# ViliamVadocz/takzero

Hardware: AMD Instinct MI355X
Metric: mcts_simulations_per_s (higher is better)
Workload: dtype f16

## Files before the change

### takzero_amd/csrc/tz_capi.hip

```cpp
#include <algorithm>
#include <array>
#include <cmath>
#include <cstdlib>
#include <cstring>
#include <vector>

#include "tz_math.h"
#include "tz_nn.h"

struct tz_search {
    SearchDev d;
    tz_net* net = nullptr;
    int device = 0;
    hipStream_t stream = nullptr;
    bool own_stream = false;
    float* noise_dev = nullptr;
    int noise_cap = 0;
    uint16_t* act_dev = nullptr;
    int32_t* i32_dev = nullptr;
    int8_t* i8_dev = nullptr;
    tz_root_info* info_dev = nullptr;
    void* child_dev = nullptr;
    size_t child_cap = 0;
    hipGraphExec_t graph[2] = {nullptr, nullptr};
// ... 66 lines not shown
int one_simulation(tz_search* s, bool from_start) {
    const int gi = from_start ? 1 : 0;
    s->sim_index++;
    const bool sample = s->profile && (s->sim_index % 8 == 0);
    if (!s->use_graph || sample || s->warm[gi] < 2) {
        s->warm[gi]++;
        return one_simulation_eager(s, from_start, sample);
    }
    if (s->graph[gi] && s->net && s->graph_gen[gi] != s->net->weights_gen) {
        (void)hipGraphExecDestroy(s->graph[gi]);
        s->graph[gi] = nullptr;
    }
    if (!s->graph[gi]) {
        hipGraph_t g = nullptr;
        TZ_HIP(hipStreamBeginCapture(s->stream, hipStreamCaptureModeThreadLocal));
        const int rc = one_simulation_eager(s, from_start, false);
        const hipError_t e = hipStreamEndCapture(s->stream, &g);
        if (rc) {
            if (g) (void)hipGraphDestroy(g);
            return rc;
        }
        if (e != hipSuccess) return tz_fail(TZ_EDEVICE, std::string("hipStreamEndCapture: ") + hipGetErrorString(e));
        const hipError_t ei = hipGraphInstantiate(&s->graph[gi], g, nullptr, nullptr, 0);
        (void)hipGraphDestroy(g);
        if (ei != hipSuccess) return tz_fail(TZ_EDEVICE, std::string("hipGraphInstantiate: ") + hipGetErrorString(ei));
        s->graph_gen[gi] = s->net ? s->net->weights_gen : 0;
    }
    TZ_HIP(hipGraphLaunch(s->graph[gi], s->stream));
    return TZ_OK;
}

int one_simulation_eager(tz_search* s, bool from_start, bool profile) {
    int rc;
    hipEvent_t e0 = nullptr, e1 = nullptr, e2 = nullptr, e3 = nullptr;
    const bool saved_net_profile = s->net ? s->net->profile : false;
    if (s->net) s->net->profile = profile;
    struct Restore {
        tz_search* s;
        bool v;
        ~Restore() {
            if (s->net) s->net->profile = v;
        }
    } restore{s, saved_net_profile};
    if (profile) {
        TZ_HIP(hipEventCreate(&e0));
        TZ_HIP(hipEventCreate(&e1));
        TZ_HIP(hipEventCreate(&e2));
        TZ_HIP(hipEventCreate(&e3));
        TZ_HIP(hipEventRecord(e0, s->stream));
    }
    if ((rc = tz_tree_descend(s->d, from_start, s->stream))) return rc;
    if ((rc = tz_tree_compact_leaves(s->d, s->stream))) return rc;
    if (profile) TZ_HIP(hipEventRecord(e1, s->stream));
    NetOut out{nullptr, 0, nullptr, nullptr};
    if (s->d.agent_kind == TZ_AGENT_NET) {
        if ((rc = tz_net_forward_device(s->net, s->d.leaf_env, s->d.nn_game, s->d.nn_count, 0, s->d.batch, s->stream, &out)))
            return rc;
    }
    if (profile) TZ_HIP(hipEventRecord(e2, s->stream));
    if ((rc = tz_tree_expand(s->d, out, s->stream))) return rc;
    if (profile) {
        TZ_HIP(hipEventRecord(e3, s->stream));
        s->tree_events.push_back({e0, e1});
        s->tree_events.push_back({e2, e3});
        s->steps++;
    }
    return TZ_OK;
}

int ensure_noise(tz_search* s, int amax) {
    if ((size_t)amax * s->d.batch <= (size_t)s->noise_cap) return TZ_OK;
    if (s->noise_dev) (void)hipFree(s->noise_dev);
    s->noise_dev = nullptr;
    TZ_HIP(hipMalloc(&s->noise_dev, (size_t)amax * s->d.batch * sizeof(float)));
    s->noise_cap = amax * s->d.batch;
    return TZ_OK;
}

void free_leaf_batch(tz_search* s) {
    LeafBatchDev& b = s->lb;
    void* ptrs[] = {b.env, b.act, b.nact, b.traj, b.traj_len, b.logit, b.prob, b.value, b.variance, b.bad, b.count, b.forwards,
                    b.offset, b.index};
    for (void* p : ptrs)
        if (p) (void)hipFree(p);
    b = LeafBatchDev{};
    s->lb_slots = 0;
}

int ensure_leaf_batch(tz_search* s, int leaves) {
    const size_t slots = (size_t)s->d.batch * leaves;
    if (slots > s->lb_slots) {
        TZ_HIP(hipStreamSynchronize(s->stream));
        free_leaf_batch(s);
        LeafBatchDev& b = s->lb;
        const size_t amax = (size_t)s->d.max_actions;
        int rc = 0;
        rc |= dev_alloc(&b.env, slots);
        rc |= dev_alloc(&b.act, slots * amax);
        rc |= dev_alloc(&b.nact, slots);
        rc |= dev_alloc(&b.traj, slots * TZ_MAX_DEPTH);
        rc |= dev_alloc(&b.traj_len, slots);
        rc |= dev_alloc(&b.logit, slots * amax);
        rc |= dev_alloc(&b.prob, slots * amax);
        rc |= dev_alloc(&b.value, slots);
        rc |= dev_alloc(&b.variance, slots);
        rc |= dev_alloc(&b.bad, slots);
        rc |= dev_alloc(&b.count, s->d.batch);
        rc |= dev_alloc(&b.forwards, s->d.batch);
        rc |= dev_alloc(&b.offset, s->d.batch);
// ... 708 lines not shown
```

### takzero_amd/csrc/tz_engine.h

```cpp
#pragma once
#include <hip/hip_runtime.h>
#include <stdint.h>

#include <string>
#include <vector>

#include "../../include/takzero_hip.h"

#define TZ_MAX_DEPTH 512

void tz_set_error(const std::string& msg);
int tz_fail(int code, const std::string& msg);
#define TZ_HIP(call)                                                                              \
    do {                                                                                          \
        hipError_t _e = (call);                                                                   \
        if (_e != hipSuccess)                                                                     \
            return tz_fail(TZ_EDEVICE, std::string(#call) + ": " + hipGetErrorString(_e));       \
    } while (0)

struct TreeArrays {
    uint8_t* eval_tag;
    uint32_t* eval_bits;
    uint32_t* visits;
    float* prob;
// ... 2 lines not shown
    uint32_t* child0;
    uint16_t* nchild;
    uint16_t* action;
};

struct SearchDev {
    int batch, n, half_komi, cap, max_actions, agent_kind;
    int strict_capacity;
    int select_rule;
    TreeArrays t;
    uint8_t* bank;
    uint32_t* alloc;
    tz_state* env;
    float* betas;
    uint32_t* traj;
    uint32_t* traj_len;
    int32_t* start_node;
    uint8_t* leaf_kind;
    uint16_t* leaf_nact;
    uint16_t* leaf_act;
    tz_state* leaf_env;
    int32_t* nn_game;
    int32_t* nn_count;
    uint32_t* bfs_src;
    unsigned long long* counters;
    int32_t* error_flag;
    int8_t* term_reason;
    uint8_t* term_winner;
};

struct LeafBatchDev {
    int leaves;
    tz_state* env;
    uint16_t* act;
    uint16_t* nact;
    uint32_t* traj;
    uint32_t* traj_len;
    float* logit;
    float* prob;
    float* value;
    float* variance;
    uint8_t* bad;
    int32_t* count;
    int32_t* forwards;
    int32_t* offset;
    int32_t* index;
};

struct NetOut {
    const float* policy;
    int policy_stride;
    const float* value;
    const float* variance;
};

int tz_tree_descend(const SearchDev& s, bool from_start_nodes, hipStream_t st);
int tz_tree_compact_leaves(const SearchDev& s, hipStream_t st);
int tz_tree_expand(const SearchDev& s, const NetOut& out, hipStream_t st);
int tz_tree_apply_noise(const SearchDev& s, const float* noise_dev, int amax, float ratio, hipStream_t st);
int tz_tree_root_info(const SearchDev& s, tz_root_info* out_dev, hipStream_t st);
int tz_tree_root_children(const SearchDev& s, int amax, uint16_t* move_idx, uint32_t* visits, uint8_t* eval_tag,
                          uint32_t* eval_bits, float* logit, float* prob, float* std_dev, hipStream_t st);
int tz_tree_node(const SearchDev& s, int game, const uint16_t* path_dev, int len, uint32_t* out_words, int* status, int amax,
                 uint16_t* move_idx, uint32_t* visits, uint8_t* eval_tag, uint32_t* eval_bits, float* logit, float* prob, float* std_dev,
                 hipStream_t st);
int tz_tree_select_best(const SearchDev& s, uint16_t* out_dev, hipStream_t st);
int tz_tree_step(const SearchDev& s, const uint16_t* actions_dev, hipStream_t st);
int tz_tree_restart(const SearchDev& s, const int32_t* choice_dev, int8_t* terminal_dev, bool force_all,
                    bool with_opening_moves, hipStream_t st);
int tz_tree_reset_games(const SearchDev& s, const int32_t* idx_dev, int count, hipStream_t st);
int tz_tree_set_start_children(const SearchDev& s, const int32_t* child_index_dev, hipStream_t st);
int tz_tree_gumbel_root_fixup(const SearchDev& s, hipStream_t st);
int tz_tree_principal_variation(const SearchDev& s, int game, uint16_t* moves_dev, int cap, int* len_dev, hipStream_t st);
int tz_tree_descend_batch(const SearchDev& s, const LeafBatchDev& b, hipStream_t st);
int tz_tree_compact_batch(const SearchDev& s, const LeafBatchDev& b, hipStream_t st);
int tz_tree_expand_batch(const SearchDev& s, const LeafBatchDev& b, const NetOut& out, hipStream_t st);
int tz_tree_play_moves(const SearchDev& s, const uint16_t* actions_dev, int8_t* ok_dev, hipStream_t st);
```

### takzero_amd/csrc/tz_nn.h

```cpp
#pragma once
#include <string>
#include <vector>

#include "tz_engine.h"
#include "tz_ot.h"

struct ConvW {
    int taps = 0, cin = 0, cin_pad = 0, cout = 0, cout_pad = 0;
    uint16_t* w_mfma = nullptr;
    uint16_t* w_lo = nullptr;
    unsigned char* w8 = nullptr;
    float c8_scale = 0.0f;
    float* w_f32 = nullptr;
    float* bias = nullptr;
};

struct tz_net {
    int n = 0, nn = 0, arch = 0, device = 0, precision = 0, blocks = 0;
    int cin = 0, cin_pad = 0, pol_ch = 0, pol_stride = 0, ppt = 0;
    bool loaded = false, has_rnd = false, has_hash = false;
    TensorStore store;
    uint64_t weights_gen = 0;
    ConvW conv_in, policy;
    std::vector<ConvW> res;
    uint16_t* tower_w = nullptr;
    uint16_t* tower_w_lo = nullptr;
    unsigned char* tower_w8 = nullptr;
    float* c8_scales = nullptr;
    float* tower_bias = nullptr;
    float* heads = nullptr;
    ConvW rnd[2][3];
    uint16_t* rndw[3] = {nullptr, nullptr, nullptr};
    float* rndb[3] = {nullptr, nullptr, nullptr};
    float rnd_min = 0.0f, rnd_max = 1.0f;
    float* simhash = nullptr;
    uint32_t* bitset = nullptr;
    int max_batch = 0;
    void *act_a = nullptr, *act_b = nullptr, *act_c = nullptr;
    float* planes = nullptr;
    float* policy_out = nullptr;
    float *value = nullptr, *ube = nullptr, *variance = nullptr, *aux = nullptr;
    void *rnd_in = nullptr, *rnd_h1 = nullptr, *rnd_h2 = nullptr;
    float* rnd_out = nullptr;
    void* seeds = nullptr;
    void* xch = nullptr;
    unsigned* xch_count = nullptr;
    bool eval_split = false;
    hipStream_t stream_rnd = nullptr;
    hipEvent_t ev_in = nullptr, ev_rnd = nullptr;
    hipStream_t stream = nullptr;
    void* dbg_buf = nullptr;
    int dbg_groups = 0;
    void* eval_host = nullptr;
    void* eval_dev = nullptr;
    size_t eval_bytes = 0;
    hipEvent_t ev0 = nullptr, ev1 = nullptr;
    std::vector<std::pair<hipEvent_t, hipEvent_t>> conv_events;
    bool profile = false;
    double conv_ms = 0.0;
    uint64_t conv_launches = 0;
};

int tz_net_ensure_batch(tz_net* net, int batch);
int tz_net_forward_device(tz_net* net, const tz_state* states_dev, const int32_t* game_index_dev,
                          const int32_t* count_dev, int count_host, int max_positions, hipStream_t st, NetOut* out);
int tz_nn_encode_planes(int n, int cin, const tz_state* states_dev, int count, float* planes_dev, hipStream_t st);
```

### takzero_amd/csrc/tz_nn.hip

```cpp
#include "tz_nn.h"
#include "tz_fp8.h"
#include "tz_fp6.h"
#include <type_traits>
#include "tz_ot.h"

#include <algorithm>
#include <cmath>
#include <cstdio>
#include <cstdlib>
#include <cstring>
#include <atomic>
#include <map>
#include <memory>
#include <mutex>
#include <thread>

int tz_nn_launch_split(int sp, int n, const void* net_args, int max_positions, hipStream_t st);
int tz_nn_launch_c6(int n, const void* net_args, int max_positions, hipStream_t st);
size_t tz_nn_c6_seed_bytes(int n, int max_positions);

namespace {

typedef float f32x4 __attribute__((ext_vector_type(4)));
typedef unsigned int u32x4 __attribute__((ext_vector_type(4)));
typedef __bf16 bf16x8 __attribute__((ext_vector_type(8)));
typedef __bf16 bf16x4 __attribute__((ext_vector_type(4)));
typedef _Float16 f16x8 __attribute__((ext_vector_type(8)));
typedef _Float16 f16x4 __attribute__((ext_vector_type(4)));

template <typename ET>
struct Elem;
template <>
struct Elem<__bf16> {
    typedef bf16x8 x8;
    typedef bf16x4 x4;
    static __device__ __forceinline__ f32x4 mfma(x8 a, x8 b, f32x4 c) { return __builtin_amdgcn_mfma_f32_16x16x32_bf16(a, b, c, 0, 0, 0); }
    static __device__ __forceinline__ __bf16 cvt(float x) { return (__bf16)x; }
    static __device__ __forceinline__ __bf16 relu_cvt(float x) { return (__bf16)(x > 0.f ? x : 0.f); }
};
template <>
struct Elem<_Float16> {
    typedef f16x8 x8;
    typedef f16x4 x4;
    static __device__ __forceinline__ f32x4 mfma(x8 a, x8 b, f32x4 c) { return __builtin_amdgcn_mfma_f32_16x16x32_f16(a, b, c, 0, 0, 0); }
    static __device__ __forceinline__ _Float16 cvt(float x) { return (_Float16)__builtin_amdgcn_fmed3f(x, -65504.0f, 65504.0f); }
    static __device__ __forceinline__ _Float16 relu_cvt(float x) { return (_Float16)__builtin_amdgcn_fmed3f(x, 0.0f, 65504.0f); }
};


constexpr int LDS_ROWB = 64;
constexpr int FILTERS = 256;
__device__ __forceinline__ int lds_piece(int row, int q) { return ((q + 2 * ((row >> 2) & 1)) & 3) << 4; }
template <int LAYOUT>
struct LdsImg {
    static constexpr int ROW_PAD = 528;
// ... 2277 lines not shown
    for (int i = l; i < out_stride; i += 64) out[(size_t)pos * out_stride + i] = (T)(i < in_size ? x[i] / ss : 0.f);
}

template <int NB, typename ET>
__global__ __launch_bounds__(64) void rnd_prep_state_kernel(const tz_state* states, const int32_t* game_index,
                                                            const int32_t* count_dev, int count_host, int cin,
                                                            int out_stride, ET* out) {
    constexpr int NN = NB * NB;
    const int count = count_dev ? *count_dev : count_host;
    const int pos = blockIdx.x, l = threadIdx.x;
    if (pos >= count) return;
    __shared__ tz_state sh;
    {
        const uint32_t* src = reinterpret_cast<const uint32_t*>(states + (game_index ? game_index[pos] : pos));
        uint32_t* dst = reinterpret_cast<uint32_t*>(&sh);
        for (int i = l; i < (int)(sizeof(tz_state) / 4); i += 64) dst[i] = src[i];
    }
    __syncthreads();
    const tz_state* s = &sh;
    const int fd = state_flat_diff<NB>(s);
    const int in_size = NN * cin;
    constexpr int PER = (NN * 40 + 63) / 64;
    float x[PER];
#pragma unroll
    for (int k = 0; k < PER; k++) {
        const int i = l + k * 64;
        x[k] = i < in_size ? plane_value<NB>(s, i / cin, i % cin, fd) : 0.f;
    }
    __shared__ float part[NN];
    if (l < NN) {
        float q = 0.f;
        for (int c = 0; c < cin; c++) {
            const float pv = plane_value<NB>(s, l, c, fd);
            q += pv * pv;
        }
        part[l] = q;
    }
    __syncthreads();
    float ss = 0.f;
    for (int sq = 0; sq < NN; sq++) ss += part[sq];
#pragma unroll
    for (int k = 0; k < PER; k++) {
        const int i = l + k * 64;
        if (i < out_stride) out[(size_t)pos * out_stride + i] = (ET)(i < in_size ? x[k] / ss : 0.f);
    }
}

__global__ __launch_bounds__(64) void rnd_finish_kernel(const float* learn, const float* target, const float* ube,
                                                        const int32_t* count_dev, int count_host, int dim, int stride,
                                                        float rmin, float rmax, float* variance) {
    const int count = count_dev ? *count_dev : count_host;
    const int pos = blockIdx.x, l = threadIdx.x;
    if (pos >= count) return;
    float s = 0.f;
    for (int i = l; i < dim; i += 64) {
        const float d = learn[(size_t)pos * stride + i] - target[(size_t)pos * stride + i];
        s += d * d;
    }
    for (int d = 32; d >= 1; d >>= 1) s += __shfl_xor(s, d);
    if (l == 0) {
        float norm = (s - rmin) / (rmax - rmin);
        norm = fminf(fmaxf(norm, 0.f), 1.f) * 4.0f;
        variance[pos] = fminf(fmaxf(fmaxf(expf(ube[pos]), norm), 0.f), 4.f);
    }
}

__global__ void plain_variance_kernel(const float* ube, const float* local, const int32_t* count_dev, int count_host,
                                      float* variance) {
    const int count = count_dev ? *count_dev : count_host;
    const int pos = blockIdx.x * blockDim.x + threadIdx.x;
    if (pos >= count) return;
    const float loc = local ? local[pos] : 0.f;
    variance[pos] = fminf(fmaxf(fmaxf(expf(ube[pos]), loc), 0.f), 4.f);
}

template <int NB>
__global__ __launch_bounds__(256) void simhash_state_kernel(const tz_state* states, const int32_t* game_index, const float* matrix,
                                                            const uint32_t* bitset, const int32_t* count_dev, int count_host, float* local,
                                                            uint32_t* index_out) {
    constexpr int NN = NB * NB, CIN = 4 * NB + 12, IN = CIN * NN, BPW = 8, DW = sizeof(tz_state) / 4;
    __shared__ tz_state st[BPW];
    __shared__ float pl[BPW][IN];
    __shared__ int fd[BPW];
    const int count = count_dev ? *count_dev : count_host;
    const int pos0 = blockIdx.x * BPW, tid = threadIdx.x;
    if (pos0 >= count) return;
    const int nb = min(BPW, count - pos0);
    for (int i = tid; i < nb * DW; i += 256) {
        const int b = i / DW, d = i - b * DW, pos = pos0 + b;
        reinterpret_cast<uint32_t*>(st)[i] = reinterpret_cast<const uint32_t*>(states + (game_index ? game_index[pos] : pos))[d];
    }
    __syncthreads();
    if (tid < nb) fd[tid] = state_flat_diff<NB>(&st[tid]);
    __syncthreads();
    for (int i = tid; i < nb * IN; i += 256) {
        const int b = i / IN, k = i - b * IN, c = k / NN, px = k - c * NN;
        pl[b][k] = c == CIN - 2 ? 0.0f : plane_value<NB>(&st[b], px, c, fd[b]);
    }
    __syncthreads();
    const int bit = tid & 31, b = tid >> 5;
    float s = 0.f;
    if (b < nb) {
#pragma unroll 8
        for (int k = 0; k < IN; k++) s += pl[b][k] * matrix[(size_t)k * 32 + bit];
    }
    const unsigned long long m = __ballot(!(s < 0.0f));
    const uint32_t index = (tid & 32) ? (uint32_t)(m >> 32) : (uint32_t)m;
    if (bit == 0 && b < nb) {
        const bool seen = bitset && ((bitset[index >> 5] >> (index & 31)) & 1u);
        local[pos0 + b] = seen ? 0.0f : 4.0f;
        if (index_out) index_out[pos0 + b] = index;
    }
}

int launch_simhash_state(int n, const tz_state* states, const int32_t* gidx, const float* matrix, const uint32_t* bitset,
                         const int32_t* count_dev, int count_host, int max_positions, float* local, uint32_t* index_out, hipStream_t st) {
    const int blocks = (max_positions + 7) / 8;
// ... 448 lines not shown
                const size_t welems = (size_t)(W.rnd[0][l].cin_pad / 32) * (W.rnd[0][l].cout_pad / 16) * 512;
                const size_t belems = W.rnd[0][l].cout_pad;
                TZ_HIP(hipMalloc(&W.rndw[l], 2 * welems * 2));
                TZ_HIP(hipMalloc(&W.rndb[l], 2 * belems * sizeof(float)));
                for (int a = 0; a < 2; a++) {
                    if ((rc = copy_sync(W.rndw[l] + a * welems, W.rnd[a][l].w_mfma, welems * 2, hipMemcpyDeviceToDevice))) return rc;
                    if ((rc = copy_sync(W.rndb[l] + a * belems, W.rnd[a][l].bias, belems * sizeof(float), hipMemcpyDeviceToDevice))) return rc;
                }
            }
        }
        if ((rc = get_tensor(m, "min", 1, t1))) return rc;
        W.rnd_min = t1[0];
        if ((rc = get_tensor(m, "max", 1, t1))) return rc;
        W.rnd_max = t1[0];
    }
    if (net->has_hash) {
        if ((rc = get_tensor(m, "simhash_matrix", (size_t)cin * nn * 32, w))) return rc;
        if ((rc = upload(w, &W.simhash))) return rc;
    }
    return TZ_OK;
}

__host__ __device__ constexpr int ppt_small(int nb) { return nb == 1 ? 64 : nb == 3 ? 7 : nb == 4 ? 6 : nb == 5 ? 4 : 3; }

int conv_cfg() {
    static int cfg = -1;
    if (cfg < 0) {
        const char* e = getenv("TZ_CONV_CFG");
        cfg = e ? atoi(e) : 0;
    }
    return cfg;
}

template <int NB, int P, int NW, int RN, int TAPS, bool FROM_STATE, bool SINGLE, int ABL = 0, int LAYOUT = 1, typename ET = __bf16, int OCC = 2>
int launch_conv(const ConvArgs& a, int max_positions, int n_blocks_y, hipStream_t st) {
    constexpr int NN = NB * NB, RT = (P * NN + 15) / 16, LROWS = RT * 16 + 8;
    const size_t smem = LdsImg<LAYOUT>::bytes(LROWS);
    auto kern = conv_mfma_kernel<NB, P, RN, TAPS, FROM_STATE, ABL, SINGLE, NW, LAYOUT, ET, OCC>;
    static bool attr_done[64] = {};
    int attr_dev = 0;
    TZ_HIP(hipGetDevice(&attr_dev));
    bool& attr_set = attr_done[attr_dev & 63];
    if (!attr_set) {
        TZ_HIP(hipFuncSetAttribute(reinterpret_cast<const void*>(kern), hipFuncAttributeMaxDynamicSharedMemorySize, (int)smem));
        attr_set = true;
    }
    dim3 grid((max_positions + P - 1) / P, n_blocks_y, a.groups > 1 ? a.groups : 1);
    hipLaunchKernelGGL(kern, grid, dim3(NW * 64), smem, st, a);
    hipError_t e = hipGetLastError();
    if (e != hipSuccess) return tz_fail(TZ_EDEVICE, std::string("conv launch: ") + hipGetErrorString(e));
    return TZ_OK;
}

int linear_grouped_bf16(int precision, const uint16_t* w, const float* bias, int groups, int cin_pad, int cout_pad, const void* in,
                        int in_stride, int in_z, void* out, int out_stride, int out_z, bool relu, bool out_f32,
                        const int32_t* count_dev, int count_host, int max_positions, hipStream_t st) {
    ConvArgs a;
    memset(&a, 0, sizeof a);
    a.in = in;
    a.count_dev = count_dev;
    a.count_host = count_host;
    a.w = w;
    a.bias = bias;
    a.out = out;
    a.cin_pad = cin_pad;
    a.kc_total = cin_pad / 32;
    a.ct_total = cout_pad / 16;
    a.out_stride = out_stride;
    a.cin_real = cin_pad;
    a.relu = relu;
    a.out_f32 = out_f32;
    a.in_stride = in_stride;
    a.groups = groups;
    a.in_z = in_z;
    a.w_z_frags = a.kc_total * a.ct_total;
    a.bias_z = cout_pad;
    a.out_z = out_z;
    if (max_positions <= 128) {
        if (prec_is_f16(precision)) return launch_conv<1, 32, 8, 2, 1, false, false, 0, 1, _Float16>(a, max_positions, cout_pad / 256, st);
        return launch_conv<1, 32, 8, 2, 1, false, false>(a, max_positions, cout_pad / 256, st);
    }
    if (prec_is_f16(precision)) return launch_conv<1, 128, 8, 2, 1, false, false, 0, 1, _Float16>(a, max_positions, cout_pad / 256, st);
    return launch_conv<1, 128, 8, 2, 1, false, false>(a, max_positions, cout_pad / 256, st);
}

template <int NB, typename ET>
int conv_board(const ConvArgs& a, int cout_pad, bool from_state, int max_positions, hipStream_t st) {
    constexpr int PA = ppt_for(NB), PB = ppt_small(NB);
    const bool wide = cout_pad % 256 == 0;
    const int by = wide ? cout_pad / 256 : cout_pad / 128;
    if (conv_cfg() == 0) {
        if (from_state) return launch_conv<NB, PA, 8, 2, 9, true, false, 0, 1, ET>(a, max_positions, by, st);
        if (wide) return launch_conv<NB, PA, 8, 2, 9, false, true, 0, 1, ET>(a, max_positions, by, st);
        return launch_conv<NB, PA, 8, 1, 9, false, true, 0, 1, ET>(a, max_positions, by, st);
    }
    if (from_state) return launch_conv<NB, PB, 4, 4, 9, true, false, 0, 1, ET>(a, max_positions, by, st);
    if (wide) return launch_conv<NB, PB, 4, 4, 9, false, true, 0, 1, ET>(a, max_positions, by, st);
    return launch_conv<NB, PB, 4, 2, 9, false, true, 0, 1, ET>(a, max_positions, by, st);
}

template <typename ET>
int conv_dispatch(int n, bool board, const ConvArgs& a, int cout_pad, bool from_state, int max_positions, hipStream_t st) {
    if (!board) return launch_conv<1, 64, 8, 2, 1, false, false, 0, 1, ET>(a, max_positions, cout_pad / 256, st);
    switch (n) {
        case 3: return conv_board<3, ET>(a, cout_pad, from_state, max_positions, st);
        case 4: return conv_board<4, ET>(a, cout_pad, from_state, max_positions, st);
        case 5: return conv_board<5, ET>(a, cout_pad, from_state, max_positions, st);
        case 6: return conv_board<6, ET>(a, cout_pad, from_state, max_positions, st);
    }
    return tz_fail(TZ_EINVAL, "conv: unsupported board size");
}

int conv_bf16(tz_net* net, const ConvW& L, const void* in, const tz_state* states, const int32_t* gidx,
              const int32_t* count_dev, int count_host, int max_positions, const void* residual, void* out,
              int out_stride, bool relu, bool out_f32, bool board, hipStream_t st) {
    ConvArgs a;
    a.in = in;
    a.states = states;
    a.game_index = gidx;
    a.count_dev = count_dev;
    a.count_host = count_host;
    a.w = L.w_mfma;
    a.bias = L.bias;
    a.residual = residual;
    a.out = out;
    a.cin_pad = L.cin_pad;
    a.kc_total = L.cin_pad / 32;
    a.ct_total = L.cout_pad / 16;
    a.out_stride = out_stride;
    a.cin_real = L.cin;
    a.relu = relu;
    a.out_f32 = out_f32;
    a.has_res = residual != nullptr;
    a.in_stride = L.cin_pad;
    a.groups = 1;
// ... 336 lines not shown
}

}

int tz_nn_encode_planes(int n, int cin, const tz_state* states_dev, int count, float* planes_dev, hipStream_t st) {
    const int total = count * n * n, blocks = (total + 127) / 128;
    switch (n) {
        case 3: encode_kernel<3><<<blocks, 128, 0, st>>>(states_dev, nullptr, nullptr, count, cin, planes_dev); break;
        case 4: encode_kernel<4><<<blocks, 128, 0, st>>>(states_dev, nullptr, nullptr, count, cin, planes_dev); break;
        case 5: encode_kernel<5><<<blocks, 128, 0, st>>>(states_dev, nullptr, nullptr, count, cin, planes_dev); break;
        case 6: encode_kernel<6><<<blocks, 128, 0, st>>>(states_dev, nullptr, nullptr, count, cin, planes_dev); break;
        default: return tz_fail(TZ_EINVAL, "encode: unsupported board size");
    }
    hipError_t e = hipGetLastError();
    if (e != hipSuccess) return tz_fail(TZ_EDEVICE, std::string("encode launch: ") + hipGetErrorString(e));
    return TZ_OK;
}

int tz_net_ensure_batch(tz_net* net, int batch) {
    if (batch <= net->max_batch) return TZ_OK;
    TZ_HIP(hipSetDevice(net->device));
    TZ_HIP(hipStreamSynchronize(net->stream));
    void** bufs[] = {&net->act_a, &net->act_b, &net->act_c, (void**)&net->planes, (void**)&net->policy_out,
                     (void**)&net->value, (void**)&net->ube, (void**)&net->variance, (void**)&net->aux,
                     &net->rnd_in, &net->rnd_h1, &net->rnd_h2, (void**)&net->rnd_out, &net->seeds};
    for (auto b : bufs) {
        if (*b) (void)hipFree(*b);
        *b = nullptr;
    }
    const size_t esz = net->precision != TZ_PREC_F32 ? 2 : 4;
    const size_t rows = (size_t)batch * net->nn;
    TZ_HIP(hipMalloc(&net->act_a, rows * FILTERS * esz));
    TZ_HIP(hipMalloc(&net->act_b, rows * FILTERS * esz));
    TZ_HIP(hipMalloc(&net->act_c, rows * FILTERS * esz));
    TZ_HIP(hipMalloc(&net->planes, rows * net->cin * sizeof(float)));
    TZ_HIP(hipMalloc(&net->policy_out, rows * net->pol_stride * sizeof(float)));
    TZ_HIP(hipMalloc(&net->value, batch * sizeof(float)));
    TZ_HIP(hipMalloc(&net->ube, batch * sizeof(float)));
    TZ_HIP(hipMalloc(&net->variance, batch * sizeof(float)));
    TZ_HIP(hipMalloc(&net->aux, batch * sizeof(float)));
    if (net->precision == TZ_PREC_F16C6) TZ_HIP(hipMalloc(&net->seeds, tz_nn_c6_seed_bytes(net->n, batch)));
    if (net->has_rnd) {
        const size_t in_pad = (size_t)(net->cin * net->nn + 31) / 32 * 32;
        TZ_HIP(hipMalloc(&net->rnd_in, (size_t)batch * in_pad * esz));
        TZ_HIP(hipMalloc(&net->rnd_h1, (size_t)batch * 2048 * esz));
        TZ_HIP(hipMalloc(&net->rnd_h2, (size_t)batch * 2048 * esz));
        TZ_HIP(hipMalloc(&net->rnd_out, (size_t)2 * batch * 512 * sizeof(float)));
    }
    net->max_batch = batch;
    return TZ_OK;
}

int tz_net_forward_device(tz_net* net, const tz_state* states, const int32_t* gidx, const int32_t* count_dev,
                          int count_host, int max_positions, hipStream_t st, NetOut* out) {
    if (!net->loaded) return tz_fail(TZ_ESTATE, "network has no weights loaded");
    if (max_positions > net->max_batch) return tz_fail(TZ_EINVAL, "forward: batch exceeds the network's buffers");
    int rc;
    const bool bf = net->precision != TZ_PREC_F32;
    const int nn = net->nn;
    const bool need_planes = !bf;
    if (need_planes && (rc = encode(net, states, gidx, count_dev, count_host, max_positions, st))) return rc;
    void *x = net->act_a, *t = net->act_b, *y = net->act_c;
    const bool split = prec_is_split(net->precision);
    const int rnd_in_pad = (net->cin * nn + 31) / 32 * 32;
    const bool rnd_ahead = net->eval_split && net->has_rnd && bf && net->n == 5 && net->stream_rnd;
    auto rnd_mlp = [&](hipStream_t rs) -> int {
        const bool fused_wrote_it = net->blocks > 0 && net->tower_w && (net_fused_mode() == 2 || split) && net_fused_writes_rnd_input(net);
        switch (net->n) {
            case 5:
                if (fused_wrote_it) break;
                if (prec_is_f16(net->precision))
                    rnd_prep_state_kernel<5, _Float16><<<max_positions, 64, 0, rs>>>(states, gidx, count_dev, count_host, net->cin, rnd_in_pad, (_Float16*)net->rnd_in);
                else
                    rnd_prep_state_kernel<5, __bf16><<<max_positions, 64, 0, rs>>>(states, gidx, count_dev, count_host, net->cin, rnd_in_pad, (__bf16*)net->rnd_in);
                break;
            default: return tz_fail(TZ_EINVAL, "RND is a net5 (5x5) feature");
        }
        float* o = net->rnd_out;
        if ((rc = linear_grouped_bf16(net->precision, net->rndw[0], net->rndb[0], 1, rnd_in_pad, 2048, net->rnd_in, rnd_in_pad, 0, net->rnd_h1, 2048, 0,
                                      true, false, count_dev, count_host, max_positions, rs)))
            return rc;
        if ((rc = linear_grouped_bf16(net->precision, net->rndw[1], net->rndb[1], 2, 1024, 1024, net->rnd_h1, 2048, 1024, net->rnd_h2, 2048, 1024,
                                      true, false, count_dev, count_host, max_positions, rs)))
            return rc;
        if ((rc = linear_grouped_bf16(net->precision, net->rndw[2], net->rndb[2], 2, 1024, 512, net->rnd_h2, 2048, 1024, o, 1024, 512, false, true,
                                      count_dev, count_host, max_positions, rs)))
            return rc;
        return TZ_OK;
    };

    if (split && !(net->blocks > 0 && (net->tower_w_lo || net->tower_w8)))
        return tz_fail(TZ_EINVAL, "forward: TZ_PREC_F16X2 / TZ_PREC_F16C8 / TZ_PREC_F16C6 need a network with at least one residual block");
    if (bf && net->blocks > 0 && net->tower_w && (net_fused_mode() == 2 || split)) {
        hipEvent_t e0 = nullptr, e1 = nullptr;
        if (net->profile) {
            TZ_HIP(hipEventCreate(&e0));
            TZ_HIP(hipEventCreate(&e1));
            TZ_HIP(hipEventRecord(e0, st));
        }
        if (rnd_ahead) {
            TZ_HIP(hipEventRecord(net->ev_in, st));
            TZ_HIP(hipStreamWaitEvent(net->stream_rnd, net->ev_in, 0));
            if ((rc = rnd_mlp(net->stream_rnd))) return rc;
            TZ_HIP(hipEventRecord(net->ev_rnd, net->stream_rnd));
        }
        if ((rc = net_fused(net, states, gidx, count_dev, count_host, max_positions, st))) return rc;
        if (net->profile) {
// ... 17 lines not shown
                TZ_HIP(hipEventRecord(e1, st));
                net->conv_events.push_back({e0, e1});
                net->conv_launches += 1;
            }
            std::swap(x, y);
        } else {
            for (int b = 0; b < net->blocks; b++) {
                hipEvent_t e0 = nullptr, e1 = nullptr;
                if (net->profile) {
                    TZ_HIP(hipEventCreate(&e0));
                    TZ_HIP(hipEventCreate(&e1));
                    TZ_HIP(hipEventRecord(e0, st));
                }
                if ((rc = conv_bf16(net, net->res[2 * b], x, nullptr, nullptr, count_dev, count_host, max_positions, nullptr, t,
                                    FILTERS, true, false, true, st)))
                    return rc;
                if ((rc = conv_bf16(net, net->res[2 * b + 1], t, nullptr, nullptr, count_dev, count_host, max_positions, x, y,
                                    FILTERS, true, false, true, st)))
                    return rc;
                if (net->profile) {
                    TZ_HIP(hipEventRecord(e1, st));
                    net->conv_events.push_back({e0, e1});
                    net->conv_launches += 2;
                }
                std::swap(x, y);
            }
        }
        if ((rc = conv_bf16(net, net->policy, x, nullptr, nullptr, count_dev, count_host, max_positions, nullptr,
                            net->policy_out, net->pol_stride, false, true, true, st)))
            return rc;
        if (prec_is_f16(net->precision))
            heads_kernel<_Float16><<<max_positions, 64, 0, st>>>((const _Float16*)x, net->heads, count_dev, count_host, nn, net->value, net->ube);
        else
            heads_kernel<__bf16><<<max_positions, 64, 0, st>>>((const __bf16*)x, net->heads, count_dev, count_host, nn, net->value, net->ube);
    } else {
        float *fx = (float*)x, *ft = (float*)t, *fy = (float*)y;
        if ((rc = conv_f32(net, net->conv_in, net->planes, net->cin, count_dev, count_host, max_positions, nullptr, fx, FILTERS,
                           true, true, st)))
            return rc;
        for (int b = 0; b < net->blocks; b++) {
            if ((rc = conv_f32(net, net->res[2 * b], fx, FILTERS, count_dev, count_host, max_positions, nullptr, ft, FILTERS, true,
                               true, st)))
                return rc;
            if ((rc = conv_f32(net, net->res[2 * b + 1], ft, FILTERS, count_dev, count_host, max_positions, fx, fy, FILTERS, true,
                               true, st)))
                return rc;
            std::swap(fx, fy);
        }
        if ((rc = conv_f32(net, net->policy, fx, FILTERS, count_dev, count_host, max_positions, nullptr, net->policy_out,
                           net->pol_stride, false, true, st)))
            return rc;
        heads_kernel<float><<<max_positions, 64, 0, st>>>(fx, net->heads, count_dev, count_host, nn, net->value, net->ube);
    }
    if (net->has_rnd) {
        const int in_size = net->cin * nn, in_pad = (in_size + 31) / 32 * 32;
        float* outs[2] = {net->rnd_out, net->rnd_out + (size_t)net->max_batch * 512};
        if (bf) {
            if (!rnd_ahead && (rc = rnd_mlp(st))) return rc;
            if (rnd_ahead) TZ_HIP(hipStreamWaitEvent(st, net->ev_rnd, 0));
            float* o = net->rnd_out;
            rnd_finish_kernel<<<max_positions, 64, 0, st>>>(o, o + 512, net->ube, count_dev, count_host, 512, 1024, net->rnd_min,
                                                            net->rnd_max, net->variance);
        } else {
            rnd_prep_kernel<float><<<max_positions, 64, 0, st>>>(net->planes, count_dev, count_host, in_size, in_pad, (float*)net->rnd_in);
            for (int a = 0; a < 2; a++) {
                if ((rc = conv_f32(net, net->rnd[a][0], (float*)net->rnd_in, in_pad, count_dev, count_host, max_positions, nullptr,
                                   (float*)net->rnd_h1, 1024, true, false, st)))
                    return rc;
                if ((rc = conv_f32(net, net->rnd[a][1], (float*)net->rnd_h1, 1024, count_dev, count_host, max_positions, nullptr,
                                   (float*)net->rnd_h2, 1024, true, false, st)))
                    return rc;
                if ((rc = conv_f32(net, net->rnd[a][2], (float*)net->rnd_h2, 1024, count_dev, count_host, max_positions, nullptr,
                                   outs[a], 512, false, false, st)))
                    return rc;
            }
        }
        if (!bf)
            rnd_finish_kernel<<<max_positions, 64, 0, st>>>(outs[0], outs[1], net->ube, count_dev, count_host, 512, 512, net->rnd_min,
                                                            net->rnd_max, net->variance);
    } else if (net->has_hash) {
        if ((rc = launch_simhash_state(net->n, states, gidx, net->simhash, net->bitset, count_dev, count_host, max_positions, net->aux, nullptr, st)))
            return rc;
        plain_variance_kernel<<<(max_positions + 255) / 256, 256, 0, st>>>(net->ube, net->aux, count_dev, count_host, net->variance);
    } else {
        plain_variance_kernel<<<(max_positions + 255) / 256, 256, 0, st>>>(net->ube, nullptr, count_dev, count_host, net->variance);
    }
    hipError_t e = hipGetLastError();
    if (e != hipSuccess) return tz_fail(TZ_EDEVICE, std::string("forward launch: ") + hipGetErrorString(e));
    out->policy = net->policy_out;
    out->policy_stride = net->pol_stride;
    out->value = net->value;
    out->variance = net->variance;
    return TZ_OK;
}

extern "C" {

int tz_device_count(void) {
    int n = 0;
    if (hipGetDeviceCount(&n) != hipSuccess) return 0;
    return n;
}

int tz_net_create(int board_n, int arch, int device_id, int precision, int blocks, tz_net** out) {
    if (!out) return tz_fail(TZ_EINVAL, "tz_net_create: null out");
    int n = board_n;
    if (arch == TZ_ARCH_NET5) n = 5;
    else if (arch == TZ_ARCH_NET4_SIMHASH) n = 4;
    else if (arch == TZ_ARCH_NET6_SIMHASH) n = 6;
    else if (arch != TZ_ARCH_TEST) return tz_fail(TZ_EINVAL, "tz_net_create: unknown architecture");
    if (board_n && board_n != n) return tz_fail(TZ_EINVAL, "tz_net_create: board size does not match the architecture");
    if (n < 3 || n > 6) return tz_fail(TZ_EINVAL, "tz_net_create: board size must be 3..6");
    if (precision != TZ_PREC_BF16 && precision != TZ_PREC_F32 && precision != TZ_PREC_F16 && precision != TZ_PREC_F16X2 && precision != TZ_PREC_F16C8 &&
        precision != TZ_PREC_F16C6)
        return tz_fail(TZ_EINVAL, "tz_net_create: bad precision");
    if (precision == TZ_PREC_F16C6 && n != 5 && n != 6) return tz_fail(TZ_EINVAL, "tz_net_create: TZ_PREC_F16C6 is built for the 5x5 and 6x6 networks");
    int ndev = 0;
    if (hipGetDeviceCount(&ndev) != hipSuccess || ndev == 0)
        return tz_fail(TZ_EDEVICE, "tz_net_create: no HIP device available (the HIP path has no CPU fallback)");
    if (device_id < 0 || device_id >= ndev) return tz_fail(TZ_EINVAL, "tz_net_create: bad device id");
    TZ_HIP(hipSetDevice(device_id));
    tz_net* net = new tz_net();
    net->n = n;
    net->nn = n * n;
    net->arch = arch;
    net->device = device_id;
    net->precision = precision;
    net->blocks = arch == TZ_ARCH_NET5 ? 20 : arch == TZ_ARCH_TEST ? blocks : 16;
    net->cin = 2 * ((3 + (n - 1) + (n + 1)) + 2) + 2;
    net->cin_pad = (net->cin + 31) / 32 * 32;
    net->pol_ch = 3 + 4 * ((1 << n) - 2);
    net->pol_stride = (net->pol_ch + 127) / 128 * 128;
    net->ppt = ppt_for(n);
    net->has_rnd = arch == TZ_ARCH_NET5;
    net->has_hash = arch == TZ_ARCH_NET4_SIMHASH || arch == TZ_ARCH_NET6_SIMHASH;
    if (hipStreamCreate(&net->stream) != hipSuccess) {
        delete net;
        return tz_fail(TZ_EDEVICE, "tz_net_create: hipStreamCreate failed");
    }
    if (net->has_hash) {
        if (hipMalloc(&net->bitset, (size_t)1 << 29) != hipSuccess || hipMemset(net->bitset, 0, (size_t)1 << 29) != hipSuccess) {
            delete net;
            return tz_fail(TZ_ENOMEM, "tz_net_create: cannot allocate the 512 MiB SimHash set");
        }
    }
// ... 839 lines not shown
```

### takzero_amd/csrc/tz_tree.hip

```cpp
#include "tz_engine.h"
#include "tz_math.h"
#include "tz_tak_dev.h"

using namespace tzd;

namespace {

struct Ev {
    uint32_t tag, bits;
};
__device__ __forceinline__ Ev ev_value(float v) { return Ev{TZ_EVAL_VALUE, tz_float_to_bits(v)}; }
__device__ __forceinline__ bool ev_known(Ev e) { return e.tag != TZ_EVAL_VALUE; }
__device__ __forceinline__ Ev ev_negate(Ev e) {
    switch (e.tag) {
        case TZ_EVAL_VALUE: return ev_value(-tz_bits_to_float(e.bits));
        case TZ_EVAL_WIN: return Ev{TZ_EVAL_LOSS, e.bits + 1};
        case TZ_EVAL_DRAW: return Ev{TZ_EVAL_DRAW, e.bits + 1};
        default: return Ev{TZ_EVAL_WIN, e.bits + 1};
    }
}
__device__ __forceinline__ float ev_to_f32(Ev e) {
    const float base = tz_powif(TZ_DISCOUNT, e.tag == TZ_EVAL_VALUE ? 0 : (int)e.bits);
    const float x = e.tag == TZ_EVAL_VALUE ? tz_bits_to_float(e.bits)
                    : e.tag == TZ_EVAL_WIN ? 1.0f
// ... 339 lines not shown
        s.traj_len[g] = (uint32_t)depth;
    }
}

__global__ __launch_bounds__(1024) void compact_kernel(SearchDev s) {
    __shared__ int wsum[16];
    __shared__ int carry;
    const int tid = threadIdx.x, l = tid & 63, w = tid >> 6;
    if (tid == 0) carry = 0;
    __syncthreads();
    for (int chunk = 0; chunk < s.batch; chunk += 1024) {
        const int g = chunk + tid;
        const int f = (g < s.batch && s.leaf_kind[g] == 1) ? 1 : 0;
        const int incl = wave_incl_scan(f);
        if (l == 63) wsum[w] = incl;
        __syncthreads();
        int off = carry;
        for (int i = 0; i < w; i++) off += wsum[i];
        if (f) s.nn_game[off + incl - 1] = g;
        __syncthreads();
        if (tid == 1023) carry = off + incl;
        __syncthreads();
    }
    if (tid == 0) {
        *s.nn_count = carry;
        s.counters[0] += (unsigned long long)s.batch;
        s.counters[1] += (unsigned long long)carry;
    }
}

template <int N>
__global__ __launch_bounds__(64) void expand_kernel(SearchDev s, NetOut out) {
    constexpr int NN = N * N;
    const int slot = blockIdx.x, l = lane_id();
    if (slot >= *s.nn_count) return;
    const int g = s.nn_game[slot];
    extern __shared__ __attribute__((aligned(16))) unsigned char smem[];
    uint32_t* tnode = reinterpret_cast<uint32_t*>(smem);
    uint32_t* tvis = tnode + TZ_MAX_DEPTH;
    float* lg = reinterpret_cast<float*>(tvis + TZ_MAX_DEPTH);
    float* ex = lg + s.max_actions;
    const size_t base = slab_base(s, s.bank[g], g);
    const int len = (int)s.traj_len[g];
    for (int i = l; i < len; i += 64) {
        const uint32_t nd = s.traj[(size_t)g * TZ_MAX_DEPTH + i];
        tnode[i] = nd;
        tvis[i] = s.t.visits[base + nd];
    }
    const int nact = s.leaf_nact[g];
    const uint16_t* acts = s.leaf_act + (size_t)g * s.max_actions;
    float value = 0.0f, variance = 0.0f;
    if (s.agent_kind == TZ_AGENT_NET) {
        value = out.value[slot];
        variance = out.variance[slot];
    } else if (s.agent_kind == TZ_AGENT_SIMPLE) {
        __shared__ tz_state le;
        load_state(&le, &s.leaf_env[g]);
        __syncthreads();
        const int fd = flat_diff<N>(&le) - s.half_komi / 2;
        value = (float)fd / (float)NN;
        if (le.to_move == 1) value = -value;
    }
    bool nan = false;
    float mx = -3.4028235e38f;
    for (int i = l; i < nact; i += 64) {
        const int a = acts[i];
        float x;
        if (s.agent_kind == TZ_AGENT_NET) {
            x = out.policy[((size_t)slot * NN + (a % NN)) * out.policy_stride + a / NN];
        } else if (s.agent_kind == TZ_AGENT_DUMMY) {
            x = 1.0f;
        } else {
            const int ch = a / NN;
            x = ch == 0 ? 4.0f : ch == 1 ? 2.0f : ch == 2 ? 3.0f : 1.0f;
        }
        nan = nan || !(x == x);
        lg[i] = x;
        mx = x > mx ? x : mx;
    }
#pragma unroll
    for (int d = 32; d >= 1; d >>= 1) {
        const float o = __shfl_xor(mx, d);
        mx = o > mx ? o : mx;
    }
    if (__any(nan) || !(value == value) || !(variance == variance)) {
        if (l == 0) atomicMax(s.error_flag, 7);
        return;
    }
    for (int i = l; i < nact; i += 64) ex[i] = tz_expf(lg[i] - mx);
    __syncthreads();
    float sum = 0.0f;
    for (int i = 0; i < nact; i++) sum = sum + ex[i];
    const uint32_t leaf = tnode[len - 1];
    const float n = (float)tvis[len - 1];
    float mean = tz_bits_to_float(s.t.eval_bits[base + leaf]);
    mean = mean + (-mean + value) / n;
    float sd = s.t.std_dev[base + leaf];
    sd = sd + (-sd + sqrtf(variance)) / n;
    const uint32_t c0 = s.alloc[g];
    const bool full = c0 + (uint32_t)nact > (uint32_t)s.cap;
    if (full && s.strict_capacity) {
        if (l == 0) atomicMax(s.error_flag, 1);
        return;
    }
    const uint32_t child_bits = tz_float_to_bits(-mean);
    for (int i = l; i < (full ? 0 : nact); i += 64) {
        const size_t ci = base + c0 + i;
// ... 818 lines not shown
```

Before: 1.451 million.

## Fuse RND variance into expand kernel and add pipelined RND linear kernel

Adds a variance_in_expand path so the search step skips the separate rnd_finish kernel and computes the RND-based variance inside the tree expand kernel from the raw RND outputs. This removes one kernel launch and a round trip through the variance buffer. It also adds a dedicated MFMA linear kernel for the RND MLP layers that double-buffers input slices in LDS and keeps a ring of prefetched weight fragments. This kernel is selected by default for large batches with matching K widths. The changes add code paths gated by an environment variable and by batch size, and the new kernel's performance depends on occupancy with its large LDS footprint.

```diff
diff --git a/takzero_amd/csrc/tz_capi.hip b/takzero_amd/csrc/tz_capi.hip
--- a/takzero_amd/csrc/tz_capi.hip
+++ b/takzero_amd/csrc/tz_capi.hip
@@ -142,9 +142,9 @@
     if ((rc = tz_tree_descend(s->d, from_start, s->stream))) return rc;
     if ((rc = tz_tree_compact_leaves(s->d, s->stream))) return rc;
     if (profile) TZ_HIP(hipEventRecord(e1, s->stream));
-    NetOut out{nullptr, 0, nullptr, nullptr};
+    NetOut out{};
     if (s->d.agent_kind == TZ_AGENT_NET) {
-        if ((rc = tz_net_forward_device(s->net, s->d.leaf_env, s->d.nn_game, s->d.nn_count, 0, s->d.batch, s->stream, &out)))
+        if ((rc = tz_net_forward_device(s->net, s->d.leaf_env, s->d.nn_game, s->d.nn_count, 0, s->d.batch, s->stream, &out, true)))
             return rc;
     }
     if (profile) TZ_HIP(hipEventRecord(e2, s->stream));
diff --git a/takzero_amd/csrc/tz_engine.h b/takzero_amd/csrc/tz_engine.h
--- a/takzero_amd/csrc/tz_engine.h
+++ b/takzero_amd/csrc/tz_engine.h
@@ -78,7 +78,29 @@
     int policy_stride;
     const float* value;
     const float* variance;
+    const float* rnd_learn;
+    const float* rnd_target;
+    int rnd_stride;
+    const float* ube;
+    float rnd_min, rnd_max;
 };
+
+constexpr int TZ_RND_DIM = 512;
+
+#if defined(__HIPCC__)
+__device__ __forceinline__ float tz_rnd_variance(const float* learn, const float* target, int dim, int l, float ube, float rmin,
+                                                 float rmax) {
+    float s = 0.f;
+    for (int i = l; i < dim; i += 64) {
+        const float d = learn[i] - target[i];
+        s = __builtin_fmaf(d, d, s);
+    }
+    for (int d = 32; d >= 1; d >>= 1) s += __shfl_xor(s, d);
+    float norm = (s - rmin) / (rmax - rmin);
+    norm = fminf(fmaxf(norm, 0.f), 1.f) * 4.0f;
+    return fminf(fmaxf(fmaxf(expf(ube), norm), 0.f), 4.f);
+}
+#endif
 
 int tz_tree_descend(const SearchDev& s, bool from_start_nodes, hipStream_t st);
 int tz_tree_compact_leaves(const SearchDev& s, hipStream_t st);
diff --git a/takzero_amd/csrc/tz_nn.h b/takzero_amd/csrc/tz_nn.h
--- a/takzero_amd/csrc/tz_nn.h
+++ b/takzero_amd/csrc/tz_nn.h
@@ -63,5 +63,6 @@
 
 int tz_net_ensure_batch(tz_net* net, int batch);
 int tz_net_forward_device(tz_net* net, const tz_state* states_dev, const int32_t* game_index_dev,
-                          const int32_t* count_dev, int count_host, int max_positions, hipStream_t st, NetOut* out);
+                          const int32_t* count_dev, int count_host, int max_positions, hipStream_t st, NetOut* out,
+                          bool variance_in_expand = false);
 int tz_nn_encode_planes(int n, int cin, const tz_state* states_dev, int count, float* planes_dev, hipStream_t st);
diff --git a/takzero_amd/csrc/tz_nn.hip b/takzero_amd/csrc/tz_nn.hip
--- a/takzero_amd/csrc/tz_nn.hip
+++ b/takzero_amd/csrc/tz_nn.hip
@@ -1,6 +1,7 @@
 #include "tz_nn.h"
 #include "tz_fp8.h"
 #include "tz_fp6.h"
+#include "tz_rnd_plan.h"
 #include <type_traits>
 #include "tz_ot.h"
 
@@ -2384,17 +2385,8 @@
     const int count = count_dev ? *count_dev : count_host;
     const int pos = blockIdx.x, l = threadIdx.x;
     if (pos >= count) return;
-    float s = 0.f;
-    for (int i = l; i < dim; i += 64) {
-        const float d = learn[(size_t)pos * stride + i] - target[(size_t)pos * stride + i];
-        s += d * d;
-    }
-    for (int d = 32; d >= 1; d >>= 1) s += __shfl_xor(s, d);
-    if (l == 0) {
-        float norm = (s - rmin) / (rmax - rmin);
-        norm = fminf(fmaxf(norm, 0.f), 1.f) * 4.0f;
-        variance[pos] = fminf(fmaxf(fmaxf(expf(ube[pos]), norm), 0.f), 4.f);
-    }
+    const float v = tz_rnd_variance(learn + (size_t)pos * stride, target + (size_t)pos * stride, dim, l, ube[pos], rmin, rmax);
+    if (l == 0) variance[pos] = v;
 }
 
 __global__ void plain_variance_kernel(const float* ube, const float* local, const int32_t* count_dev, int count_host,
@@ -2949,6 +2941,167 @@
     return TZ_OK;
 }
 
+template <int P, int KC, typename ET>
+__global__ __launch_bounds__(512) void rnd_linear_kernel(ConvArgs a) {
+    typedef typename Elem<ET>::x8 ex8;
+    typedef typename Elem<ET>::x4 ex4;
+    constexpr int NW = 8, NT = NW * 64, RN = 2, RT = P / 16, LROWS = P + 8;
+    constexpr int PLANE = LROWS * LDS_ROWB, BUF = TZ_RND_SLICE_MAX * PLANE;
+    constexpr int NLOAD = P * 32 / NT;
+    constexpr int RING = P >= 128 ? 4 : 8;
+    static_assert(P % 16 == 0 && NLOAD * NT == P * 32 && (RT - 1) * 16 * LDS_ROWB < 65536, "tile");
+    extern __shared__ __attribute__((aligned(16))) unsigned char lds[];
+    const int count = a.count_dev ? *a.count_dev : a.count_host;
+    const int pos0 = blockIdx.x * P;
+    if (pos0 >= count) return;
+    const int tid = threadIdx.x, lane = tid & 63;
+    const int wave = __builtin_amdgcn_readfirstlane(tid >> 6);
+    const int q = lane >> 4, lr = lane & 15;
+    const int valid_rows = min(P, count - pos0);
+    constexpr int kc_total = KC, nslices = tz_rnd_slice_count(KC);
+    const int ct0 = (blockIdx.y * NW + wave) * RN;
+    const __amdgpu_buffer_rsrc_t wrsrc = __builtin_amdgcn_make_buffer_rsrc(
+        const_cast<uint16_t*>(a.w), 0, (a.groups > 1 ? a.groups * a.w_z_frags : kc_total * a.ct_total) * 1024, 0x00020000);
+    const int lane16 = lane * 16;
+    auto wload = [&](int kcg, int j) -> ex8 {
+        const int frag = (int)blockIdx.z * a.w_z_frags + kcg * a.ct_total + (ct0 + j);
+        const u32x4 r = __builtin_amdgcn_raw_buffer_load_b128(wrsrc, lane16, frag * 1024, 0);
+        return __builtin_bit_cast(ex8, r);
+    };
+    const uint16_t* in = reinterpret_cast<const uint16_t*>(a.in) + (size_t)blockIdx.z * a.in_z + (size_t)pos0 * a.in_stride;
+    const __amdgpu_buffer_rsrc_t irsrc = __builtin_amdgcn_make_buffer_rsrc(
+        const_cast<uint16_t*>(in), 0, ((valid_rows - 1) * a.in_stride + a.cin_pad) * 2, 0x00020000);
+    auto fetch = [&](int s, uint4 (&v)[NLOAD]) {
+        const int c0 = tz_rnd_slice_start(kc_total, s) * 64, pieces = tz_rnd_slice_len(kc_total, s) * 4;
+#pragma unroll
+        for (int i = 0; i < NLOAD; i++) {
+            const int id = tid + i * NT, row = id >> 5, ci = id & 31;
+            const int off = row * a.in_stride * 2 + c0 + ci * 16;
+            const u32x4 r = __builtin_amdgcn_raw_buffer_load_b128(irsrc, row < valid_rows && ci < pieces ? off : (int)0x80000000, 0, 0);
+            v[i] = __builtin_bit_cast(uint4, r);
+        }
+    };
+    auto stash = [&](int s, const uint4 (&v)[NLOAD]) {
+        unsigned char* buf = lds + (s & 1) * BUF;
+#pragma unroll
+        for (int i = 0; i < NLOAD; i++) {
+            const int id = tid + i * NT, row = id >> 5, ci = id & 31;
+            *reinterpret_cast<uint4*>(buf + LdsImg<1>::store_addr(row, ci, PLANE)) = v[i];
+        }
+    };
+
+    uint4 stage[NLOAD];
+    ex8 bq[RING][RN];
+    {
+        uint4 first[NLOAD];
+        fetch(0, first);
+        if (nslices > 1) fetch(1, stage);
+#pragma unroll
+        for (int k = 0; k < RING - 1; k++)
+            if (k < kc_total) {
+#pragma unroll
+                for (int j = 0; j < RN; j++) bq[k][j] = wload(k, j);
+            }
+        stash(0, first);
+        if (nslices > 1) stash(1, stage);
+        if (nslices > 2) fetch(2, stage);
+    }
+    __syncthreads();
+    f32x4 acc[RT][RN];
+#pragma unroll
+    for (int rt = 0; rt < RT; rt++)
+#pragma unroll
+        for (int j = 0; j < RN; j++) acc[rt][j] = f32x4{0.f, 0.f, 0.f, 0.f};
+    const int abase = lr * LDS_ROWB + lds_piece(lr, q);
+    ex8 av[RT];
+#pragma unroll
+    for (int rt = 0; rt < RT; rt++) av[rt] = *reinterpret_cast<const ex8*>(lds + abase + rt * 16 * LDS_ROWB);
+    int s = 0, last = tz_rnd_slice_len(kc_total, 0) - 1;
+    int cur = 0;
+#pragma unroll
+    for (int g = 0; g < KC; g++) {
+        if (g + RING - 1 < KC) {
+#pragma unroll
+            for (int j = 0; j < RN; j++) bq[(g + RING - 1) % RING][j] = wload(g + RING - 1, j);
+        }
+        __builtin_amdgcn_sched_barrier(0);
+        const bool ends = g == last && s + 1 < nslices;
+        if (ends) {
+            __syncthreads();
+            if (s + 2 < nslices) {
+                stash(s + 2, stage);
+                if (s + 3 < nslices) fetch(s + 3, stage);
+            }
+        }
+        const int nxt = ends ? ((s + 1) & 1) * BUF : cur + PLANE;
+#pragma unroll
+        for (int rt = 0; rt < RT; rt++) {
+#pragma unroll
+            for (int j = 0; j < RN; j++) acc[rt][j] = Elem<ET>::mfma(bq[g % RING][j], av[rt], acc[rt][j]);
+            if (g + 1 < KC) av[rt] = *reinterpret_cast<const ex8*>(lds + abase + nxt + rt * 16 * LDS_ROWB);
+        }
+        if (ends) {
+            s++;
+            last += tz_rnd_slice_len(kc_total, s);
+        }
+        cur = nxt;
+    }
+
+#pragma unroll
+    for (int j = 0; j < RN; j++) {
+        const int cbase = (ct0 + j) * 16 + q * 4;
+        const f32x4 bias = *reinterpret_cast<const f32x4*>(a.bias + (size_t)blockIdx.z * a.bias_z + cbase);
+#pragma unroll
+        for (int rt = 0; rt < RT; rt++) {
+            const int r = rt * 16 + lr;
+            if (r >= valid_rows) continue;
+            f32x4 v = acc[rt][j] + bias;
+            const size_t o = (size_t)blockIdx.z * a.out_z + (size_t)(pos0 + r) * a.out_stride + cbase;
+            if (a.relu) {
+#pragma unroll
+                for (int k = 0; k < 4; k++) v[k] = v[k] > 0.f ? v[k] : 0.f;
+            }
+            if (a.out_f32) {
+                *reinterpret_cast<f32x4*>(reinterpret_cast<float*>(a.out) + o) = v;
+            } else {
+                ex4 ov;
+#pragma unroll
+                for (int k = 0; k < 4; k++) ov[k] = Elem<ET>::cvt(v[k]);
+                *reinterpret_cast<ex4*>(reinterpret_cast<uint16_t*>(a.out) + o) = ov;
+            }
+        }
+    }
+}
+
+template <int P, int KC, typename ET>
+int launch_rnd_linear(const ConvArgs& a, int max_positions, int n_blocks_y, hipStream_t st) {
+    constexpr size_t smem = (size_t)2 * TZ_RND_SLICE_MAX * (P + 8) * LDS_ROWB;
+    static_assert(smem <= 160 * 1024, "two slice buffers fit the CU's LDS");
+    auto kern = rnd_linear_kernel<P, KC, ET>;
+    static bool attr_done[64] = {};
+    int attr_dev = 0;
+    TZ_HIP(hipGetDevice(&attr_dev));
+    bool& attr_set = attr_done[attr_dev & 63];
+    if (!attr_set) {
+        TZ_HIP(hipFuncSetAttribute(reinterpret_cast<const void*>(kern), hipFuncAttributeMaxDynamicSharedMemorySize, (int)smem));
+        attr_set = true;
+    }
+    dim3 grid((max_positions + P - 1) / P, n_blocks_y, a.groups > 1 ? a.groups : 1);
+    hipLaunchKernelGGL(kern, grid, dim3(512), smem, st, a);
+    hipError_t e = hipGetLastError();
+    if (e != hipSuccess) return tz_fail(TZ_EDEVICE, std::string("rnd linear launch: ") + hipGetErrorString(e));
+    return TZ_OK;
+}
+
+int rnd_linear_mode() {
+    static const int mode = [] {
+        const char* e = getenv("TZ_RND_LINEAR");
+        return !e ? 0 : !strcmp(e, "conv") ? 1 : !strcmp(e, "conv4") ? 2 : 0;
+    }();
+    return mode;
+}
+bool rnd_linear_shipped() { return rnd_linear_mode() == 1; }
+
 int linear_grouped_bf16(int precision, const uint16_t* w, const float* bias, int groups, int cin_pad, int cout_pad, const void* in,
                         int in_stride, int in_z, void* out, int out_stride, int out_z, bool relu, bool out_f32,
                         const int32_t* count_dev, int count_host, int max_positions, hipStream_t st) {
@@ -2977,7 +3130,22 @@
         if (prec_is_f16(precision)) return launch_conv<1, 32, 8, 2, 1, false, false, 0, 1, _Float16>(a, max_positions, cout_pad / 256, st);
         return launch_conv<1, 32, 8, 2, 1, false, false>(a, max_positions, cout_pad / 256, st);
     }
-    if (prec_is_f16(precision)) return launch_conv<1, 128, 8, 2, 1, false, false, 0, 1, _Float16>(a, max_positions, cout_pad / 256, st);
+    const bool f16 = prec_is_f16(precision);
+    if (max_positions > 256 && rnd_linear_mode() == 0) {
+        const bool narrow = cout_pad * (groups > 1 ? groups : 1) < 2048;
+        const int by = cout_pad / 256;
+        if (a.kc_total == 25 && !narrow)
+            return f16 ? launch_rnd_linear<128, 25, _Float16>(a, max_positions, by, st) : launch_rnd_linear<128, 25, __bf16>(a, max_positions, by, st);
+        if (a.kc_total == 32 && !narrow)
+            return f16 ? launch_rnd_linear<128, 32, _Float16>(a, max_positions, by, st) : launch_rnd_linear<128, 32, __bf16>(a, max_positions, by, st);
+        if (a.kc_total == 32 && narrow)
+            return f16 ? launch_rnd_linear<64, 32, _Float16>(a, max_positions, by, st) : launch_rnd_linear<64, 32, __bf16>(a, max_positions, by, st);
+    }
+    if (max_positions > 256 && rnd_linear_mode() == 2) {
+        if (f16) return launch_conv<1, 128, 4, 2, 1, false, false, 0, 1, _Float16>(a, max_positions, cout_pad / 128, st);
+        return launch_conv<1, 128, 4, 2, 1, false, false>(a, max_positions, cout_pad / 128, st);
+    }
+    if (f16) return launch_conv<1, 128, 8, 2, 1, false, false, 0, 1, _Float16>(a, max_positions, cout_pad / 256, st);
     return launch_conv<1, 128, 8, 2, 1, false, false>(a, max_positions, cout_pad / 256, st);
 }
 
@@ -3420,7 +3588,7 @@
 }
 
 int tz_net_forward_device(tz_net* net, const tz_state* states, const int32_t* gidx, const int32_t* count_dev,
-                          int count_host, int max_positions, hipStream_t st, NetOut* out) {
+                          int count_host, int max_positions, hipStream_t st, NetOut* out, bool variance_in_expand) {
     if (!net->loaded) return tz_fail(TZ_ESTATE, "network has no weights loaded");
     if (max_positions > net->max_batch) return tz_fail(TZ_EINVAL, "forward: batch exceeds the network's buffers");
     int rc;
@@ -3544,6 +3712,7 @@
             return rc;
         heads_kernel<float><<<max_positions, 64, 0, st>>>(fx, net->heads, count_dev, count_host, nn, net->value, net->ube);
     }
+    bool finish_in_expand = false;
     if (net->has_rnd) {
         const int in_size = net->cin * nn, in_pad = (in_size + 31) / 32 * 32;
         float* outs[2] = {net->rnd_out, net->rnd_out + (size_t)net->max_batch * 512};
@@ -3551,8 +3720,10 @@
             if (!rnd_ahead && (rc = rnd_mlp(st))) return rc;
             if (rnd_ahead) TZ_HIP(hipStreamWaitEvent(st, net->ev_rnd, 0));
             float* o = net->rnd_out;
-            rnd_finish_kernel<<<max_positions, 64, 0, st>>>(o, o + 512, net->ube, count_dev, count_host, 512, 1024, net->rnd_min,
-                                                            net->rnd_max, net->variance);
+            finish_in_expand = variance_in_expand && !rnd_ahead && !rnd_linear_shipped();
+            if (!finish_in_expand)
+                rnd_finish_kernel<<<max_positions, 64, 0, st>>>(o, o + TZ_RND_DIM, net->ube, count_dev, count_host, TZ_RND_DIM, 1024, net->rnd_min,
+                                                                net->rnd_max, net->variance);
         } else {
             rnd_prep_kernel<float><<<max_positions, 64, 0, st>>>(net->planes, count_dev, count_host, in_size, in_pad, (float*)net->rnd_in);
             for (int a = 0; a < 2; a++) {
@@ -3583,6 +3754,12 @@
     out->policy_stride = net->pol_stride;
     out->value = net->value;
     out->variance = net->variance;
+    out->rnd_learn = finish_in_expand ? net->rnd_out : nullptr;
+    out->rnd_target = finish_in_expand ? net->rnd_out + TZ_RND_DIM : nullptr;
+    out->rnd_stride = finish_in_expand ? 1024 : 0;
+    out->ube = finish_in_expand ? net->ube : nullptr;
+    out->rnd_min = finish_in_expand ? net->rnd_min : 0.f;
+    out->rnd_max = finish_in_expand ? net->rnd_max : 0.f;
     return TZ_OK;
 }
 
diff --git a/takzero_amd/csrc/tz_rnd_plan.h b/takzero_amd/csrc/tz_rnd_plan.h
--- /dev/null
+++ b/takzero_amd/csrc/tz_rnd_plan.h
@@ -0,0 +1,21 @@
+#pragma once
+
+#if defined(__HIPCC__) || defined(__CUDACC__)
+#define TZ_RND_PLAN_FN __host__ __device__ inline constexpr
+#else
+#define TZ_RND_PLAN_FN inline constexpr
+#endif
+
+constexpr int TZ_RND_SLICE_MAX = 8;
+
+TZ_RND_PLAN_FN int tz_rnd_slice_count(int kc_total) { return (kc_total + TZ_RND_SLICE_MAX - 1) / TZ_RND_SLICE_MAX; }
+
+TZ_RND_PLAN_FN int tz_rnd_slice_len(int kc_total, int s) {
+    const int n = tz_rnd_slice_count(kc_total);
+    return kc_total / n + (s < kc_total % n ? 1 : 0);
+}
+
+TZ_RND_PLAN_FN int tz_rnd_slice_start(int kc_total, int s) {
+    const int n = tz_rnd_slice_count(kc_total), base = kc_total / n, rem = kc_total % n;
+    return s * base + (s < rem ? s : rem);
+}
diff --git a/takzero_amd/csrc/tz_tree.hip b/takzero_amd/csrc/tz_tree.hip
--- a/takzero_amd/csrc/tz_tree.hip
+++ b/takzero_amd/csrc/tz_tree.hip
@@ -415,7 +415,11 @@
     float value = 0.0f, variance = 0.0f;
     if (s.agent_kind == TZ_AGENT_NET) {
         value = out.value[slot];
-        variance = out.variance[slot];
+        if (out.rnd_learn)
+            variance = tz_rnd_variance(out.rnd_learn + (size_t)slot * out.rnd_stride, out.rnd_target + (size_t)slot * out.rnd_stride,
+                                       TZ_RND_DIM, l, out.ube[slot], out.rnd_min, out.rnd_max);
+        else
+            variance = out.variance[slot];
     } else if (s.agent_kind == TZ_AGENT_SIMPLE) {
         __shared__ tz_state le;
         load_state(&le, &s.leaf_env[g]);
```

After: 1.454 million (median of 3 runs). Within noise of the previous version (+0.2%).
